# Merricx/zksnake

Hardware: AMD Instinct MI355X
Metric: BN254 G1 MSM throughput (higher is better)
Workload: dtype u32 limbs (254-bit modular integers)

## Files before the change

### zksnake_amd/csrc/curve.hip.h

```cpp
#pragma once
#include "field.hip.h"

namespace zkmi {

template <class F>
struct Affine {
    typename F::T x, y;
};

template <class F>
struct XYZZ {
    typename F::T X, Y, ZZ, ZZZ;
};

template <class F>
ZK_HD bool aff_is_inf(const Affine<F>& p) {
    return F::is_zero(p.x) && F::is_zero(p.y);
}

template <class F>
ZK_HD Affine<F> aff_neg(const Affine<F>& p) {
    return {p.x, F::neg(p.y)};
}

template <class F>
ZK_HD XYZZ<F> xyzz_inf() {
    return {F::zero(), F::zero(), F::zero(), F::zero()};
}

template <class F>
ZK_HD bool xyzz_is_inf(const XYZZ<F>& p) {
    return F::is_zero(p.ZZ);
}

template <class F>
ZK_HD XYZZ<F> xyzz_from_affine(const Affine<F>& p) {
    if (aff_is_inf<F>(p)) return xyzz_inf<F>();
    return {p.x, p.y, F::one(), F::one()};
}

template <class F>
ZK_HD XYZZ<F> xyzz_neg(const XYZZ<F>& p) {
    return {p.X, F::neg(p.Y), p.ZZ, p.ZZZ};
}

template <class F>
ZK_HD XYZZ<F> xyzz_dbl_affine(const Affine<F>& p) {
    typedef typename F::T T;
    if (aff_is_inf<F>(p) || F::is_zero(p.y)) return xyzz_inf<F>();
    T U = F::dbl(p.y);
    T V = F::sqr(U);
    T W = F::mul(U, V);
    T S = F::mul(p.x, V);
    T xx = F::sqr(p.x);
    T M = F::add(F::dbl(xx), xx);
    T X3 = F::sub(F::sqr(M), F::dbl(S));
    T Y3 = F::mul_diff(M, S, X3, W, p.y);
    return {X3, Y3, V, W};
}

template <class F>
ZK_HD XYZZ<F> xyzz_dbl(const XYZZ<F>& p) {
    typedef typename F::T T;
    if (xyzz_is_inf<F>(p) || F::is_zero(p.Y)) return xyzz_inf<F>();
    T U = F::dbl(p.Y);
    T V = F::sqr(U);
    T W = F::mul(U, V);
    T S = F::mul(p.X, V);
    T xx = F::sqr(p.X);
    T M = F::add(F::dbl(xx), xx);
    T X3 = F::sub(F::sqr(M), F::dbl(S));
    T Y3 = F::mul_diff(M, S, X3, W, p.Y);
    T ZZ3 = F::mul(V, p.ZZ);
    T ZZZ3 = F::mul(W, p.ZZZ);
    return {X3, Y3, ZZ3, ZZZ3};
}

template <class F>
ZK_HD void xyzz_add_affine(XYZZ<F>& acc, const Affine<F>& q) {
    typedef typename F::T T;
    if (aff_is_inf<F>(q)) return;
    if (xyzz_is_inf<F>(acc)) {
        acc = {q.x, q.y, F::one(), F::one()};
        return;
    }
    T U2 = F::mul(q.x, acc.ZZ);
    T S2 = F::mul(q.y, acc.ZZZ);
    T Pd = F::sub(U2, acc.X);
    T R = F::sub(S2, acc.Y);
    if (F::is_zero(Pd)) {
        if (F::is_zero(R)) acc = xyzz_dbl_affine<F>(q);
        else acc = xyzz_inf<F>();
        return;
    }
    T PP = F::sqr(Pd);
    T PPP = F::mul(Pd, PP);
    T Q = F::mul(acc.X, PP);
    T X3 = F::sub(F::sub(F::sqr(R), PPP), F::dbl(Q));
    T Y3 = F::mul_diff(R, Q, X3, acc.Y, PPP);
    acc.X = X3;
    acc.Y = Y3;
    acc.ZZ = F::mul(acc.ZZ, PP);
    acc.ZZZ = F::mul(acc.ZZZ, PPP);
}

template <class F>
ZK_HD void xyzz_add_affine_relaxed2(XYZZ<F>& acc, const Affine<F>& q, bool negate) {
    typedef typename F::T T;
    typedef typename F::Params P;
    if (F::is_zero_limbs(q.x) && F::is_zero_limbs(q.y)) return;
    if (F::is_zero_limbs(acc.ZZ)) {
        acc = {q.x, negate ? F::neg(q.y) : q.y, F::one(), F::one()};
        return;
    }
    const T U2 = fp2_mul_relaxed<P, 4>(q.x, acc.ZZ);
    T ny = {fp_sub_k<P, 2>(fp_zero<P>(), q.y.c0), fp_sub_k<P, 2>(fp_zero<P>(), q.y.c1)};
#pragma unroll
    for (int i = 0; i < P::N; ++i) {
        ny.c0.v[i] = negate ? ny.c0.v[i] : q.y.c0.v[i];
        ny.c1.v[i] = negate ? ny.c1.v[i] : q.y.c1.v[i];
    }
    const T S2 = fp2_mul_relaxed<P, 4>(ny, acc.ZZZ);
    const T Pd = {fp_sub_k<P, 4>(U2.c0, acc.X.c0), fp_sub_k<P, 4>(U2.c1, acc.X.c1)};
    const T R = {fp_sub_k<P, 2>(S2.c0, acc.Y.c0), fp_sub_k<P, 2>(S2.c1, acc.Y.c1)};
    const T PP = fp2_sqr_relaxed<P, 8>(Pd);
    const T RR = fp2_sqr_relaxed<P, 4>(R);
    if (fp_is_zero<P>(PP.c0) && fp_is_zero<P>(PP.c1)) {
        if (fp_is_zero<P>(RR.c0) && fp_is_zero<P>(RR.c1)) {
            Affine<F> d = q;
            if (negate) d.y = F::neg(d.y);
            acc = xyzz_dbl_affine<F>(d);
        } else {
            acc = xyzz_inf<F>();
        }
        return;
    }
    const T PPP = fp2_mul_relaxed<P, 8>(Pd, PP);
    const T Q = fp2_mul_relaxed<P, 8>(acc.X, PP);
    const T X3 = {fp_sub_twice_sel4<P>(fp_sub_k<P, 2>(RR.c0, PPP.c0), Q.c0), fp_sub_twice_sel4<P>(fp_sub_k<P, 2>(RR.c1, PPP.c1), Q.c1)};
    const T D = {fp_sub_k<P, 4>(Q.c0, X3.c0), fp_sub_k<P, 4>(Q.c1, X3.c1)};
    if constexpr (P::N <= 9) {
        const Fp<P> nR1 = fp_neg_lazy_k<P, 8>(R.c1), nY0 = fp_neg_lazy_k<P, 4>(acc.Y.c0), nY1 = fp_neg_lazy_k<P, 4>(acc.Y.c1);
        acc.Y = {fp_mul4<P>(R.c0, D.c0, nR1, D.c1, nY0, PPP.c0, acc.Y.c1, PPP.c1),
                 fp_mul4<P>(R.c0, D.c1, nY0, PPP.c1, nY1, PPP.c0, R.c1, D.c0)};
    } else {
        acc.Y = fp2_sub<P>(fp2_mul_relaxed<P, 8>(R, D), fp2_mul_relaxed<P, 4>(acc.Y, PPP));
    }
    acc.X = X3;
    acc.ZZ = fp2_mul_relaxed<P, 4>(acc.ZZ, PP);
    acc.ZZZ = fp2_mul_relaxed<P, 4>(acc.ZZZ, PPP);
}

template <class F>
ZK_HD void xyzz_relaxed_finish(XYZZ<F>& acc) {
    if constexpr (F::RELAXED2) {
        typedef typename F::Params P;
        acc.X = {fp_reduce_2p<P>(acc.X.c0), fp_reduce_2p<P>(acc.X.c1)};
    }
}

#if defined(__HIPCC__)
template <class F>
__device__ __forceinline__ Affine<F> load_affine_row(const uint32_t* p) {
    uint32_t w[2 * F::LIMBS];
    const uint4* q = reinterpret_cast<const uint4*>(p);
#pragma unroll
    for (int i = 0; i < 2 * F::LIMBS / 4; ++i) {
        uint4 t = q[i];
        w[4 * i] = t.x; w[4 * i + 1] = t.y; w[4 * i + 2] = t.z; w[4 * i + 3] = t.w;
    }
    return {F::load(w), F::load(w + F::LIMBS)};
}

template <class F>
__device__ __forceinline__ void xyzz_add_affine_mem(XYZZ<F>& acc, const uint32_t* src, bool negate) {
    typedef typename F::T T;
    if constexpr (F::RELAXED) {
        T U2, S2;
        {
            Affine<F> q = load_affine_row<F>(src);
            if (F::is_zero_limbs(q.x) && F::is_zero_limbs(q.y)) return;
            if (F::is_zero_limbs(acc.ZZ)) {
                acc = {q.x, negate ? F::neg(q.y) : q.y, F::one(), F::one()};
                return;
            }
            U2 = F::mul(q.x, acc.ZZ);
            T ny = F::neg_for_mul(q.y);
#pragma unroll
            for (int i = 0; i < F::REGS; ++i) ny.v[i] = negate ? ny.v[i] : q.y.v[i];
            S2 = F::mul(ny, acc.ZZZ);
        }
        T Pd = F::template sub_k<4>(U2, acc.X);
        T R = F::template sub_k<2>(S2, acc.Y);
        T PP = F::sqr(Pd);
        T RR = F::sqr(R);
        if (F::is_zero(PP)) {
            if (F::is_zero(RR)) {
                Affine<F> q = load_affine_row<F>(src);
                if (negate) q.y = F::neg(q.y);
                acc = xyzz_dbl_affine<F>(q);
            } else {
                acc = xyzz_inf<F>();
            }
            return;
        }
        T PPP = F::mul(Pd, PP);
        T Q = F::mul(acc.X, PP);
        T X3 = F::x3_sel4(F::template sub_k<2>(RR, PPP), Q);
        acc.Y = F::y3_relaxed(R, Q, X3, acc.Y, PPP);
        acc.X = X3;
        acc.ZZ = F::mul(acc.ZZ, PP);
        acc.ZZZ = F::mul(acc.ZZZ, PPP);
    } else if constexpr (F::RELAXED2) {
        xyzz_add_affine_relaxed2<F>(acc, load_affine_row<F>(src), negate);
    } else {
        T U2, S2;
        {
            Affine<F> q = load_affine_row<F>(src);
            if (F::is_zero_limbs(q.x) && F::is_zero_limbs(q.y)) return;
            if (negate) q.y = F::neg(q.y);
            if (F::is_zero_limbs(acc.ZZ)) {
                acc = {q.x, q.y, F::one(), F::one()};
                return;
            }
            U2 = F::mul(q.x, acc.ZZ);
            S2 = F::mul(q.y, acc.ZZZ);
        }
        T Pd = F::sub(U2, acc.X);
        T R = F::sub(S2, acc.Y);
        if (F::is_zero(Pd)) {
            if (F::is_zero(R)) {
                Affine<F> q = load_affine_row<F>(src);
                if (negate) q.y = F::neg(q.y);
                acc = xyzz_dbl_affine<F>(q);
            } else {
                acc = xyzz_inf<F>();
            }
            return;
        }
        T PP = F::sqr(Pd);
        T PPP = F::mul(Pd, PP);
        T Q = F::mul(acc.X, PP);
        T X3 = F::sub(F::sub(F::sqr(R), PPP), F::dbl(Q));
        acc.Y = F::mul_diff(R, Q, X3, acc.Y, PPP);
        acc.X = X3;
        acc.ZZ = F::mul(acc.ZZ, PP);
        acc.ZZZ = F::mul(acc.ZZZ, PPP);
    }
}
#endif

template <class F>
ZK_HD XYZZ<F> xyzz_add(const XYZZ<F>& p, const XYZZ<F>& q) {
    typedef typename F::T T;
    if (xyzz_is_inf<F>(q)) return p;
    if (xyzz_is_inf<F>(p)) return q;
    T U1 = F::mul(p.X, q.ZZ);
    T U2 = F::mul(q.X, p.ZZ);
    T S1 = F::mul(p.Y, q.ZZZ);
    T S2 = F::mul(q.Y, p.ZZZ);
    T Pd = F::sub(U2, U1);
    T R = F::sub(S2, S1);
    if (F::is_zero(Pd)) {
        if (F::is_zero(R)) return xyzz_dbl<F>(p);
        return xyzz_inf<F>();
    }
    T PP = F::sqr(Pd);
    T PPP = F::mul(Pd, PP);
    T Q = F::mul(U1, PP);
    T X3 = F::sub(F::sub(F::sqr(R), PPP), F::dbl(Q));
    T Y3 = F::mul_diff(R, Q, X3, S1, PPP);
    T ZZ3 = F::mul(F::mul(p.ZZ, q.ZZ), PP);
    T ZZZ3 = F::mul(F::mul(p.ZZZ, q.ZZZ), PPP);
    return {X3, Y3, ZZ3, ZZZ3};
}

template <class F>
ZK_HD Affine<F> xyzz_to_affine(const XYZZ<F>& p) {
    typedef typename F::T T;
    if (xyzz_is_inf<F>(p)) return {F::zero(), F::zero()};
    T inv = F::inv(F::mul(p.ZZ, p.ZZZ));
    T izz = F::mul(inv, p.ZZZ);
    T izzz = F::mul(inv, p.ZZ);
    return {F::mul(p.X, izz), F::mul(p.Y, izzz)};
}

template <class F>
ZK_HD XYZZ<F> xyzz_scalar_mul(const Affine<F>& p, const uint32_t* k, int nlimbs) {
    XYZZ<F> acc = xyzz_inf<F>();
    bool started = false;
    for (int i = nlimbs * 32 - 1; i >= 0; --i) {
        if (started) acc = xyzz_dbl<F>(acc);
        if ((k[i >> 5] >> (i & 31)) & 1) {
            xyzz_add_affine<F>(acc, p);
            started = true;
        }
    }
    return acc;
}

template <class F>
ZK_HD bool aff_on_curve(const Affine<F>& p, const typename F::T& b) {
    if (aff_is_inf<F>(p)) return true;
    typename F::T lhs = F::sqr(p.y);
    typename F::T rhs = F::add(F::mul(F::sqr(p.x), p.x), b);
    return F::eq(lhs, rhs);
}

}
```

### zksnake_amd/csrc/fp2_split.hip.h

```cpp
#pragma once
#include "pair.hip.h"

namespace zkmi {

template <class P>
struct SplitXYZZ {
    Fp<P> X, Y, ZZ, ZZZ;
};

template <class P>
__device__ __forceinline__ Fp<P> sp_sel(bool odd, const Fp<P>& even_v, const Fp<P>& odd_v) {
    Fp<P> r;
#pragma unroll
    for (int i = 0; i < P::N; ++i) r.v[i] = odd ? odd_v.v[i] : even_v.v[i];
    return r;
}

template <class P, int K>
__device__ __forceinline__ Fp<P> sp_mul(const Fp<P>& a, const Fp<P>& b, bool odd) {
    const Fp<P> xa = pair_xch<Fp<P>>(a), xb = pair_xch<Fp<P>>(b);
    const Fp<P> nxa = fp_neg_lazy_k<P, K>(xa);
    return fp_mul2<P>(sp_sel<P>(odd, a, xa), b, sp_sel<P>(odd, nxa, a), xb);
}

template <class P, int KD>
__device__ __forceinline__ Fp<P> sp_sqr(const Fp<P>& a, bool odd) {
    const Fp<P> xa = pair_xch<Fp<P>>(a);
    const Fp<P> ts = fp_add_nosel<P>(a, xa);
    const Fp<P> td = fp_sub_k<P, KD>(a, xa);
    return fp_mul<P>(sp_sel<P>(odd, ts, fp_dbl_lazy<P>(xa)), sp_sel<P>(odd, td, a));
}

template <class P>
__device__ __forceinline__ Fp<P> sp_sqr_plain(const Fp<P>& a, bool odd) {
    const Fp<P> xa = pair_xch<Fp<P>>(a);
    const Fp<P> prod = fp_mul<P>(sp_sel<P>(odd, fp_add<P>(a, xa), xa), sp_sel<P>(odd, fp_sub<P>(a, xa), a));
    return sp_sel<P>(odd, prod, fp_dbl<P>(prod));
}

template <class P>
__device__ __forceinline__ bool sp_is_zero(const Fp<P>& a) {
    const bool z = fp_is_zero<P>(a);
    return pair_xch_flag(z) && z;
}
template <class P>
__device__ __forceinline__ bool sp_is_zero_limbs(const Fp<P>& a) {
    const bool z = fp_is_zero_limbs<P>(a);
    return pair_xch_flag(z) && z;
}

template <class P>
__device__ __forceinline__ SplitXYZZ<P> sp_inf() {
    return {fp_zero<P>(), fp_zero<P>(), fp_zero<P>(), fp_zero<P>()};
}

template <class P>
__device__ __forceinline__ SplitXYZZ<P> sp_dbl_affine(const Fp<P>& x, const Fp<P>& y, bool odd) {
    if (sp_is_zero<P>(y)) return sp_inf<P>();
    const Fp<P> U = fp_dbl<P>(y);
    const Fp<P> V = sp_sqr_plain<P>(U, odd);
    const Fp<P> W = sp_mul<P, 4>(U, V, odd);
    const Fp<P> S = sp_mul<P, 4>(x, V, odd);
    const Fp<P> xx = sp_sqr_plain<P>(x, odd);
    const Fp<P> M = fp_add<P>(fp_dbl<P>(xx), xx);
    const Fp<P> X3 = fp_sub<P>(sp_sqr_plain<P>(M, odd), fp_dbl<P>(S));
    const Fp<P> Y3 = fp_sub<P>(sp_mul<P, 4>(M, fp_sub<P>(S, X3), odd), sp_mul<P, 4>(W, y, odd));
    return {X3, Y3, V, W};
}

template <class P>
__device__ __forceinline__ void sp_add_affine(SplitXYZZ<P>& acc, const Fp<P>& qx, const Fp<P>& qy, bool negate, bool odd) {
    {
        const bool qz = fp_is_zero_limbs<P>(qx) && fp_is_zero_limbs<P>(qy);
        if (pair_xch_flag(qz) && qz) return;
    }
    if (sp_is_zero_limbs<P>(acc.ZZ)) {
        const Fp<P> one = sp_sel<P>(odd, fp_one<P>(), fp_zero<P>());
        acc = {qx, negate ? fp_neg<P>(qy) : qy, one, one};
        return;
    }
    const Fp<P> U2 = sp_mul<P, 4>(qx, acc.ZZ, odd);
    Fp<P> ny = fp_sub_k<P, 2>(fp_zero<P>(), qy);
#pragma unroll
    for (int i = 0; i < P::N; ++i) ny.v[i] = negate ? ny.v[i] : qy.v[i];
    const Fp<P> S2 = sp_mul<P, 4>(ny, acc.ZZZ, odd);
    const Fp<P> Pd = fp_sub_k<P, 4>(U2, acc.X);
    const Fp<P> R = fp_sub_k<P, 2>(S2, acc.Y);
    const Fp<P> PP = sp_sqr<P, 8>(Pd, odd);
    const Fp<P> RR = sp_sqr<P, 4>(R, odd);
    if (sp_is_zero<P>(PP)) {
        if (sp_is_zero<P>(RR)) acc = sp_dbl_affine<P>(qx, negate ? fp_neg<P>(qy) : qy, odd);
        else acc = sp_inf<P>();
        return;
    }
    const Fp<P> PPP = sp_mul<P, 8>(Pd, PP, odd);
    const Fp<P> Q = sp_mul<P, 8>(acc.X, PP, odd);
    const Fp<P> X3 = fp_sub_twice_sel4<P>(fp_sub_k<P, 2>(RR, PPP), Q);
    const Fp<P> D = fp_sub_k<P, 4>(Q, X3);
    if constexpr (P::N <= 9) {
        const Fp<P> xR = pair_xch<Fp<P>>(R), xD = pair_xch<Fp<P>>(D), xY = pair_xch<Fp<P>>(acc.Y), xP = pair_xch<Fp<P>>(PPP);
        const Fp<P> nY = fp_neg_lazy_k<P, 4>(acc.Y), nxY = fp_neg_lazy_k<P, 4>(xY), nxR = fp_neg_lazy_k<P, 8>(xR);
        acc.Y = fp_mul4<P>(sp_sel<P>(odd, R, xR), D, sp_sel<P>(odd, nxR, R), xD, sp_sel<P>(odd, nY, nxY), PPP, sp_sel<P>(odd, xY, nY), xP);
    } else {
        acc.Y = fp_sub<P>(sp_mul<P, 8>(R, D, odd), sp_mul<P, 4>(acc.Y, PPP, odd));
    }
    acc.X = X3;
    acc.ZZ = sp_mul<P, 4>(acc.ZZ, PP, odd);
    acc.ZZZ = sp_mul<P, 4>(acc.ZZZ, PPP, odd);
}

}
```

### zksnake_amd/csrc/msm_accumulate.hip.h

```cpp
#pragma once
#include "msm_common.hip.h"
#include "fp2_split.hip.h"
#ifndef ZK_SPLIT_WAVES_BN
#define ZK_SPLIT_WAVES_BN 3
#endif
#ifndef ZK_SPLIT_WAVES_BLS
#define ZK_SPLIT_WAVES_BLS 1
#endif

namespace zkmi {


template <class F>
__device__ __forceinline__ uint32_t* run_slot(uint32_t* partials, uint32_t* buckets, const uint32_t* run_start, const uint32_t* bucket_start,
                                              uint32_t key, uint32_t t, uint32_t seg_len) {
    constexpr int XW = 4 * F::LIMBS;
    const uint32_t r0 = run_start[key];
    if (run_start[key + 1] - r0 == 1) return buckets + (size_t)key * XW;
    return partials + (size_t)(r0 + t - bucket_start[key] / seg_len) * XW;
}

template <class G> struct AccumulateWaves { static constexpr int PER_SIMD = 1; };
template <> struct AccumulateWaves<Bn254G2> { static constexpr int PER_SIMD = 2; };

template <class G>
__global__ __launch_bounds__(256, AccumulateWaves<G>::PER_SIMD) void accumulate_kernel(const uint32_t* __restrict__ bases,
                                                         const uint32_t* __restrict__ sorted,
                                                         const uint32_t* __restrict__ bucket_start,
                                                         const uint32_t* __restrict__ run_start, uint32_t n_keys,
                                                         uint32_t seg_len, uint32_t prio_steps, uint32_t* __restrict__ partials,
                                                         uint32_t* __restrict__ buckets) {
    typedef typename G::F F;
    constexpr int AW = 2 * F::LIMBS;
    const uint32_t t = blockIdx.x * blockDim.x + threadIdx.x;
    const uint32_t total = bucket_start[n_keys];
    const uint32_t begin = t * seg_len;
    if (begin >= total) return;
    uint32_t end = begin + seg_len;
    if (end > total) end = total;
    uint32_t lo = 0, hi = n_keys;
    while (hi - lo > 1) {
        uint32_t mid = (lo + hi) >> 1;
        if (bucket_start[mid] <= begin) lo = mid; else hi = mid;
    }
    uint32_t key = lo;
    uint32_t next = bucket_start[key + 1];
    XYZZ<F> acc = xyzz_inf<F>();
    const uint32_t q1 = seg_len - seg_len / 4, q2 = seg_len - seg_len / 10, q3 = seg_len - (seg_len + 31) / 32;
    if (prio_steps) __builtin_amdgcn_s_setprio(3);
    for (uint32_t e = begin; e < end; ++e) {
        if (prio_steps) {
            const uint32_t step = __builtin_amdgcn_readfirstlane(e - begin);
            if (step == q1) __builtin_amdgcn_s_setprio(2);
            else if (step == q2) __builtin_amdgcn_s_setprio(1);
            else if (step == q3) __builtin_amdgcn_s_setprio(0);
        }
        if (e == next) {
            xyzz_relaxed_finish<F>(acc);
            store_xyzz<F>(run_slot<F>(partials, buckets, run_start, bucket_start, key, t, seg_len), acc);
            acc = xyzz_inf<F>();
            do {
                ++key;
                next = bucket_start[key + 1];
            } while (next <= e);
        }
        uint32_t ref = sorted[e];
        const uint32_t* src = bases + (size_t)(ref & 0x7FFFFFFFu) * AW;
        xyzz_add_affine_mem<F>(acc, src, (ref >> 31) != 0);
    }
    xyzz_relaxed_finish<F>(acc);
    store_xyzz<F>(run_slot<F>(partials, buckets, run_start, bucket_start, key, t, seg_len), acc);
}

template <class G> struct AccumulateSplit { static constexpr bool ON = false; static constexpr bool DEFAULT = false; static constexpr int WAVES = 1; };
template <> struct AccumulateSplit<Bn254G2> { static constexpr bool ON = true; static constexpr bool DEFAULT = false; static constexpr int WAVES = ZK_SPLIT_WAVES_BN; };
template <> struct AccumulateSplit<Bls381G2> { static constexpr bool ON = true; static constexpr bool DEFAULT = true; static constexpr int WAVES = ZK_SPLIT_WAVES_BLS; };

template <class P>
__device__ __forceinline__ Fp<P> load_component(const uint32_t* p) {
    uint32_t w[P::W];
    load_words<P::W>(w, p);
    return fp_load<P>(w);
}
template <class P>
__device__ __forceinline__ void store_split_xyzz(uint32_t* row, bool odd, const SplitXYZZ<P>& a) {
    constexpr int W = P::W;
    uint32_t w[W];
    uint32_t* base = row + (odd ? W : 0);
    fp_store<P>(w, a.X);   store_words<W>(base, w);
    fp_store<P>(w, a.Y);   store_words<W>(base + 2 * W, w);
    fp_store<P>(w, a.ZZ);  store_words<W>(base + 4 * W, w);
    fp_store<P>(w, a.ZZZ); store_words<W>(base + 6 * W, w);
}

template <class G>
__global__ __launch_bounds__(256, AccumulateSplit<G>::WAVES) void accumulate_split_kernel(const uint32_t* __restrict__ bases,
                                                         const uint32_t* __restrict__ sorted,
                                                         const uint32_t* __restrict__ bucket_start,
                                                         const uint32_t* __restrict__ run_start, uint32_t n_keys,
                                                         uint32_t seg_len, uint32_t prio_steps, uint32_t* __restrict__ partials,
                                                         uint32_t* __restrict__ buckets) {
    typedef typename G::F F;
    typedef typename F::Params P;
    constexpr int W = P::W;
    constexpr int AW = 4 * W;
    const uint32_t gt = blockIdx.x * blockDim.x + threadIdx.x;
    const uint32_t t = gt >> 1;
    const bool odd = (gt & 1) != 0;
    const uint32_t total = bucket_start[n_keys];
    const uint32_t begin = t * seg_len;
    if (begin >= total) return;
    uint32_t end = begin + seg_len;
    if (end > total) end = total;
    uint32_t lo = 0, hi = n_keys;
    while (hi - lo > 1) {
        uint32_t mid = (lo + hi) >> 1;
        if (bucket_start[mid] <= begin) lo = mid; else hi = mid;
    }
    uint32_t key = lo;
    uint32_t next = bucket_start[key + 1];
    SplitXYZZ<P> acc = sp_inf<P>();
    const uint32_t q1 = seg_len - seg_len / 4, q2 = seg_len - seg_len / 10, q3 = seg_len - (seg_len + 31) / 32;
    if (prio_steps) __builtin_amdgcn_s_setprio(3);
    for (uint32_t e = begin; e < end; ++e) {
        if (prio_steps) {
            const uint32_t step = __builtin_amdgcn_readfirstlane(e - begin);
            if (step == q1) __builtin_amdgcn_s_setprio(2);
            else if (step == q2) __builtin_amdgcn_s_setprio(1);
            else if (step == q3) __builtin_amdgcn_s_setprio(0);
        }
        if (e == next) {
            acc.X = fp_reduce_2p<P>(acc.X);
            store_split_xyzz<P>(run_slot<F>(partials, buckets, run_start, bucket_start, key, t, seg_len), odd, acc);
            acc = sp_inf<P>();
            do {
                ++key;
                next = bucket_start[key + 1];
            } while (next <= e);
        }
        const uint32_t ref = sorted[e];
        const uint32_t* src = bases + (size_t)(ref & 0x7FFFFFFFu) * AW + (odd ? W : 0);
        const Fp<P> qx = load_component<P>(src), qy = load_component<P>(src + 2 * W);
        sp_add_affine<P>(acc, qx, qy, (ref >> 31) != 0, odd);
    }
    acc.X = fp_reduce_2p<P>(acc.X);
    store_split_xyzz<P>(run_slot<F>(partials, buckets, run_start, bucket_start, key, t, seg_len), odd, acc);
}


template <class G>
__global__ void bases_to_mont_kernel(const uint32_t* __restrict__ in, uint64_t n, uint32_t* __restrict__ out, int glv) {
    typedef typename G::F F;
    constexpr int AW = 2 * F::LIMBS;
    uint64_t i = (uint64_t)blockIdx.x * blockDim.x + threadIdx.x;
    if (i >= n) return;
    uint32_t w[AW];
    load_words<AW>(w, in + i * AW);
    Affine<F> p;
    p.x = F::from_canonical(w);
    p.y = F::from_canonical(w + F::LIMBS);
    if constexpr (GlvOf<G>::OK) {
        if (glv) {
            typedef typename F::Params FP;
            store_affine<F>(out + 2 * i * AW, p);
            const Fp<FP> beta = fp_from_canonical<FP>(GlvOf<G>::P::BETA);
            if constexpr (GlvOf<G>::P::NEG_Y) {
                p.x = {fp_mul<FP>(p.x.c0, beta), fp_mul<FP>(p.x.c1, beta)};
                p.y = F::neg(p.y);
            } else {
                p.x = fp_mul<FP>(p.x, beta);
            }
            store_affine<F>(out + (2 * i + 1) * AW, p);
            return;
        }
    }
    store_affine<F>(out + i * AW, p);
}

}
```

Measured before the change: 712.3.

## Wave-cooperative bucket search, tracked empty flag, and cheaper run-slot selection in accumulate

Replaces the per-thread binary search over bucket_start with a wave-cooperative 64-way ballot search followed by a shuffle refinement, so the lanes of a wave share memory probes. Replaces the per-add zero test on the accumulator's ZZ limbs with a register boolean that tracks whether the accumulator is empty. Computes the run offset once and derives whether the run is single-segment from it, which removes two global loads per bucket flush. Together these cut serial latency and global loads in the accumulate kernels. The cost is more complex control flow and some risk around edge cases such as the one-run test at segment ends.

```diff
diff --git a/zksnake_amd/csrc/curve.hip.h b/zksnake_amd/csrc/curve.hip.h
--- a/zksnake_amd/csrc/curve.hip.h
+++ b/zksnake_amd/csrc/curve.hip.h
@@ -105,12 +105,13 @@
 }
 
 template <class F>
-ZK_HD void xyzz_add_affine_relaxed2(XYZZ<F>& acc, const Affine<F>& q, bool negate) {
+ZK_HD void xyzz_add_affine_relaxed2(XYZZ<F>& acc, const Affine<F>& q, bool negate, bool& empty) {
     typedef typename F::T T;
     typedef typename F::Params P;
     if (F::is_zero_limbs(q.x) && F::is_zero_limbs(q.y)) return;
-    if (F::is_zero_limbs(acc.ZZ)) {
+    if (empty) {
         acc = {q.x, negate ? F::neg(q.y) : q.y, F::one(), F::one()};
+        empty = false;
         return;
     }
     const T U2 = fp2_mul_relaxed<P, 4>(q.x, acc.ZZ);
@@ -130,8 +131,10 @@
             Affine<F> d = q;
             if (negate) d.y = F::neg(d.y);
             acc = xyzz_dbl_affine<F>(d);
+            empty = F::is_zero_limbs(acc.ZZ);
         } else {
             acc = xyzz_inf<F>();
+            empty = true;
         }
         return;
     }
@@ -152,6 +155,12 @@
 }
 
 template <class F>
+ZK_HD void xyzz_add_affine_relaxed2(XYZZ<F>& acc, const Affine<F>& q, bool negate) {
+    bool empty = F::is_zero_limbs(acc.ZZ);
+    xyzz_add_affine_relaxed2<F>(acc, q, negate, empty);
+}
+
+template <class F>
 ZK_HD void xyzz_relaxed_finish(XYZZ<F>& acc) {
     if constexpr (F::RELAXED2) {
         typedef typename F::Params P;
@@ -173,15 +182,16 @@
 }
 
 template <class F>
-__device__ __forceinline__ void xyzz_add_affine_mem(XYZZ<F>& acc, const uint32_t* src, bool negate) {
+__device__ __forceinline__ void xyzz_add_affine_mem(XYZZ<F>& acc, const uint32_t* src, bool negate, bool& empty) {
     typedef typename F::T T;
     if constexpr (F::RELAXED) {
         T U2, S2;
         {
             Affine<F> q = load_affine_row<F>(src);
             if (F::is_zero_limbs(q.x) && F::is_zero_limbs(q.y)) return;
-            if (F::is_zero_limbs(acc.ZZ)) {
+            if (empty) {
                 acc = {q.x, negate ? F::neg(q.y) : q.y, F::one(), F::one()};
+                empty = false;
                 return;
             }
             U2 = F::mul(q.x, acc.ZZ);
@@ -199,8 +209,10 @@
                 Affine<F> q = load_affine_row<F>(src);
                 if (negate) q.y = F::neg(q.y);
                 acc = xyzz_dbl_affine<F>(q);
+                empty = F::is_zero_limbs(acc.ZZ);
             } else {
                 acc = xyzz_inf<F>();
+                empty = true;
             }
             return;
         }
@@ -212,15 +224,16 @@
         acc.ZZ = F::mul(acc.ZZ, PP);
         acc.ZZZ = F::mul(acc.ZZZ, PPP);
     } else if constexpr (F::RELAXED2) {
-        xyzz_add_affine_relaxed2<F>(acc, load_affine_row<F>(src), negate);
+        xyzz_add_affine_relaxed2<F>(acc, load_affine_row<F>(src), negate, empty);
     } else {
         T U2, S2;
         {
             Affine<F> q = load_affine_row<F>(src);
             if (F::is_zero_limbs(q.x) && F::is_zero_limbs(q.y)) return;
             if (negate) q.y = F::neg(q.y);
-            if (F::is_zero_limbs(acc.ZZ)) {
+            if (empty) {
                 acc = {q.x, q.y, F::one(), F::one()};
+                empty = false;
                 return;
             }
             U2 = F::mul(q.x, acc.ZZ);
@@ -233,8 +246,10 @@
                 Affine<F> q = load_affine_row<F>(src);
                 if (negate) q.y = F::neg(q.y);
                 acc = xyzz_dbl_affine<F>(q);
+                empty = F::is_zero_limbs(acc.ZZ);
             } else {
                 acc = xyzz_inf<F>();
+                empty = true;
             }
             return;
         }
@@ -247,6 +262,11 @@
         acc.ZZ = F::mul(acc.ZZ, PP);
         acc.ZZZ = F::mul(acc.ZZZ, PPP);
     }
+}
+template <class F>
+__device__ __forceinline__ void xyzz_add_affine_mem(XYZZ<F>& acc, const uint32_t* src, bool negate) {
+    bool empty = F::is_zero_limbs(acc.ZZ);
+    xyzz_add_affine_mem<F>(acc, src, negate, empty);
 }
 #endif
 
diff --git a/zksnake_amd/csrc/fp2_split.hip.h b/zksnake_amd/csrc/fp2_split.hip.h
--- a/zksnake_amd/csrc/fp2_split.hip.h
+++ b/zksnake_amd/csrc/fp2_split.hip.h
@@ -69,14 +69,15 @@
 }
 
 template <class P>
-__device__ __forceinline__ void sp_add_affine(SplitXYZZ<P>& acc, const Fp<P>& qx, const Fp<P>& qy, bool negate, bool odd) {
+__device__ __forceinline__ void sp_add_affine(SplitXYZZ<P>& acc, const Fp<P>& qx, const Fp<P>& qy, bool negate, bool odd, bool& empty) {
     {
         const bool qz = fp_is_zero_limbs<P>(qx) && fp_is_zero_limbs<P>(qy);
         if (pair_xch_flag(qz) && qz) return;
     }
-    if (sp_is_zero_limbs<P>(acc.ZZ)) {
+    if (empty) {
         const Fp<P> one = sp_sel<P>(odd, fp_one<P>(), fp_zero<P>());
         acc = {qx, negate ? fp_neg<P>(qy) : qy, one, one};
+        empty = false;
         return;
     }
     const Fp<P> U2 = sp_mul<P, 4>(qx, acc.ZZ, odd);
@@ -89,8 +90,13 @@
     const Fp<P> PP = sp_sqr<P, 8>(Pd, odd);
     const Fp<P> RR = sp_sqr<P, 4>(R, odd);
     if (sp_is_zero<P>(PP)) {
-        if (sp_is_zero<P>(RR)) acc = sp_dbl_affine<P>(qx, negate ? fp_neg<P>(qy) : qy, odd);
-        else acc = sp_inf<P>();
+        if (sp_is_zero<P>(RR)) {
+            acc = sp_dbl_affine<P>(qx, negate ? fp_neg<P>(qy) : qy, odd);
+            empty = sp_is_zero_limbs<P>(acc.ZZ);
+        } else {
+            acc = sp_inf<P>();
+            empty = true;
+        }
         return;
     }
     const Fp<P> PPP = sp_mul<P, 8>(Pd, PP, odd);
@@ -108,5 +114,10 @@
     acc.ZZ = sp_mul<P, 4>(acc.ZZ, PP, odd);
     acc.ZZZ = sp_mul<P, 4>(acc.ZZZ, PPP, odd);
 }
+template <class P>
+__device__ __forceinline__ void sp_add_affine(SplitXYZZ<P>& acc, const Fp<P>& qx, const Fp<P>& qy, bool negate, bool odd) {
+    bool empty = sp_is_zero_limbs<P>(acc.ZZ);
+    sp_add_affine<P>(acc, qx, qy, negate, odd, empty);
+}
 
 }
diff --git a/zksnake_amd/csrc/msm_accumulate.hip.h b/zksnake_amd/csrc/msm_accumulate.hip.h
--- a/zksnake_amd/csrc/msm_accumulate.hip.h
+++ b/zksnake_amd/csrc/msm_accumulate.hip.h
@@ -12,12 +12,44 @@
 
 
 template <class F>
-__device__ __forceinline__ uint32_t* run_slot(uint32_t* partials, uint32_t* buckets, const uint32_t* run_start, const uint32_t* bucket_start,
-                                              uint32_t key, uint32_t t, uint32_t seg_len) {
+__device__ __forceinline__ uint32_t* run_slot(uint32_t* partials, uint32_t* buckets, const uint32_t* run_start, uint32_t key, uint32_t run_off,
+                                              bool one_run) {
     constexpr int XW = 4 * F::LIMBS;
-    const uint32_t r0 = run_start[key];
-    if (run_start[key + 1] - r0 == 1) return buckets + (size_t)key * XW;
-    return partials + (size_t)(r0 + t - bucket_start[key] / seg_len) * XW;
+    if (one_run) return buckets + (size_t)key * XW;
+    return partials + (size_t)(run_start[key] + run_off) * XW;
+}
+
+__device__ __forceinline__ uint32_t first_key_of_segment(const uint32_t* __restrict__ bucket_start, uint32_t n_keys, uint32_t begin,
+                                                         uint32_t wave_begin, bool live) {
+    const uint32_t lane = threadIdx.x & 63u;
+    uint32_t lo = 0, span = n_keys;
+    while (span > 1) {
+        const uint32_t step = (span + 63u) >> 6;
+        const uint32_t probe = lo + (lane + 1u) * step;
+        const bool le = probe < lo + span && bucket_start[probe] <= wave_begin;
+        const uint32_t cnt = (uint32_t)__popcll(__ballot(le));
+        const uint32_t hi = lo + span;
+        lo += cnt * step;
+        span = hi - lo < step ? hi - lo : step;
+    }
+    const uint32_t wi = lo + 1u + lane;
+    const uint32_t wv = wi < n_keys ? bucket_start[wi] : 0xFFFFFFFFu;
+    uint32_t c = 0;
+#pragma unroll
+    for (uint32_t b = 64; b; b >>= 1) {
+        const uint32_t i = c + b - 1u;
+        const uint32_t v = (uint32_t)__shfl((int)wv, (int)(i & 63u), 64);
+        if (i < 64u && v <= begin) c += b;
+    }
+    uint32_t key = lo + c;
+    if (live && c == 64u) {
+        uint32_t hi = n_keys;
+        while (hi - key > 1) {
+            uint32_t mid = (key + hi) >> 1;
+            if (bucket_start[mid] <= begin) key = mid; else hi = mid;
+        }
+    }
+    return key;
 }
 
 template <class G> struct AccumulateWaves { static constexpr int PER_SIMD = 1; };
@@ -35,16 +67,15 @@
     const uint32_t t = blockIdx.x * blockDim.x + threadIdx.x;
     const uint32_t total = bucket_start[n_keys];
     const uint32_t begin = t * seg_len;
+    const uint32_t wave_begin = __builtin_amdgcn_readfirstlane(begin);
+    if (wave_begin >= total) return;
+    uint32_t key = first_key_of_segment(bucket_start, n_keys, begin, wave_begin, begin < total);
     if (begin >= total) return;
     uint32_t end = begin + seg_len;
     if (end > total) end = total;
-    uint32_t lo = 0, hi = n_keys;
-    while (hi - lo > 1) {
-        uint32_t mid = (lo + hi) >> 1;
-        if (bucket_start[mid] <= begin) lo = mid; else hi = mid;
-    }
-    uint32_t key = lo;
     uint32_t next = bucket_start[key + 1];
+    uint32_t run_off = t - bucket_start[key] / seg_len;
+    bool empty = true;
     XYZZ<F> acc = xyzz_inf<F>();
     const uint32_t q1 = seg_len - seg_len / 4, q2 = seg_len - seg_len / 10, q3 = seg_len - (seg_len + 31) / 32;
     if (prio_steps) __builtin_amdgcn_s_setprio(3);
@@ -56,9 +87,11 @@
             else if (step == q3) __builtin_amdgcn_s_setprio(0);
         }
         if (e == next) {
+            if (empty) acc = xyzz_inf<F>();
             xyzz_relaxed_finish<F>(acc);
-            store_xyzz<F>(run_slot<F>(partials, buckets, run_start, bucket_start, key, t, seg_len), acc);
-            acc = xyzz_inf<F>();
+            store_xyzz<F>(run_slot<F>(partials, buckets, run_start, key, run_off, run_off == 0), acc);
+            empty = true;
+            run_off = 0;
             do {
                 ++key;
                 next = bucket_start[key + 1];
@@ -66,10 +99,11 @@
         }
         uint32_t ref = sorted[e];
         const uint32_t* src = bases + (size_t)(ref & 0x7FFFFFFFu) * AW;
-        xyzz_add_affine_mem<F>(acc, src, (ref >> 31) != 0);
-    }
+        xyzz_add_affine_mem<F>(acc, src, (ref >> 31) != 0, empty);
+    }
+    if (empty) acc = xyzz_inf<F>();
     xyzz_relaxed_finish<F>(acc);
-    store_xyzz<F>(run_slot<F>(partials, buckets, run_start, bucket_start, key, t, seg_len), acc);
+    store_xyzz<F>(run_slot<F>(partials, buckets, run_start, key, run_off, run_off == 0 && next <= end), acc);
 }
 
 template <class G> struct AccumulateSplit { static constexpr bool ON = false; static constexpr bool DEFAULT = false; static constexpr int WAVES = 1; };
@@ -109,16 +143,15 @@
     const bool odd = (gt & 1) != 0;
     const uint32_t total = bucket_start[n_keys];
     const uint32_t begin = t * seg_len;
+    const uint32_t wave_begin = __builtin_amdgcn_readfirstlane(begin);
+    if (wave_begin >= total) return;
+    uint32_t key = first_key_of_segment(bucket_start, n_keys, begin, wave_begin, begin < total);
     if (begin >= total) return;
     uint32_t end = begin + seg_len;
     if (end > total) end = total;
-    uint32_t lo = 0, hi = n_keys;
-    while (hi - lo > 1) {
-        uint32_t mid = (lo + hi) >> 1;
-        if (bucket_start[mid] <= begin) lo = mid; else hi = mid;
-    }
-    uint32_t key = lo;
     uint32_t next = bucket_start[key + 1];
+    uint32_t run_off = t - bucket_start[key] / seg_len;
+    bool empty = true;
     SplitXYZZ<P> acc = sp_inf<P>();
     const uint32_t q1 = seg_len - seg_len / 4, q2 = seg_len - seg_len / 10, q3 = seg_len - (seg_len + 31) / 32;
     if (prio_steps) __builtin_amdgcn_s_setprio(3);
@@ -130,9 +163,11 @@
             else if (step == q3) __builtin_amdgcn_s_setprio(0);
         }
         if (e == next) {
+            if (empty) acc = sp_inf<P>();
             acc.X = fp_reduce_2p<P>(acc.X);
-            store_split_xyzz<P>(run_slot<F>(partials, buckets, run_start, bucket_start, key, t, seg_len), odd, acc);
-            acc = sp_inf<P>();
+            store_split_xyzz<P>(run_slot<F>(partials, buckets, run_start, key, run_off, run_off == 0), odd, acc);
+            empty = true;
+            run_off = 0;
             do {
                 ++key;
                 next = bucket_start[key + 1];
@@ -141,10 +176,11 @@
         const uint32_t ref = sorted[e];
         const uint32_t* src = bases + (size_t)(ref & 0x7FFFFFFFu) * AW + (odd ? W : 0);
         const Fp<P> qx = load_component<P>(src), qy = load_component<P>(src + 2 * W);
-        sp_add_affine<P>(acc, qx, qy, (ref >> 31) != 0, odd);
-    }
+        sp_add_affine<P>(acc, qx, qy, (ref >> 31) != 0, odd, empty);
+    }
+    if (empty) acc = sp_inf<P>();
     acc.X = fp_reduce_2p<P>(acc.X);
-    store_split_xyzz<P>(run_slot<F>(partials, buckets, run_start, bucket_start, key, t, seg_len), odd, acc);
+    store_split_xyzz<P>(run_slot<F>(partials, buckets, run_start, key, run_off, run_off == 0 && next <= end), odd, acc);
 }
 
 
```

Result: no change. 717.2, median of 6 (+0.7%).
